# bmhopkinson/hyslam

Measured on AMD Instinct MI355X. Metric: stereo frames/sec ORB extract+match, 1920x1080 @2000 feat, higher is better.
Workload: dtype u8

## Files before the change

hyslam_amd/csrc/hs_api.hip:

```cpp
#include "hs_plan.h"
#include "hs_track.h"
#include <atomic>
#include <climits>
#include <cmath>
#include <cstdio>
#include <cstring>
#include <mutex>
#include <string>
#include <vector>

#define HS_VERSION "hyslam_amd 0.1 (gfx950)"

template <class T, bool Pinned = false> struct HsBuf {
    T* p = nullptr; size_t cap = 0;
    HsBuf() = default;
    HsBuf(const HsBuf&) = delete; HsBuf& operator=(const HsBuf&) = delete;
    HsBuf(HsBuf&& o) noexcept : p(o.p), cap(o.cap) { o.p = nullptr; o.cap = 0; }
    HsBuf& operator=(HsBuf&& o) noexcept { if (this != &o) { release(); p = o.p; cap = o.cap; o.p = nullptr; o.cap = 0; } return *this; }
    ~HsBuf() { release(); }
    void release() { if (p) (void)(Pinned ? hipHostFree(p) : hipFree(p)); p = nullptr; cap = 0; }
    hipError_t grow(size_t count)
    {
        if (count <= cap) return hipSuccess;
        release();
        const hipError_t e = Pinned ? hipHostMalloc((void**)&p, count * sizeof(T), hipHostMallocDefault) : hipMalloc((void**)&p, count * sizeof(T));
        if (e != hipSuccess) { p = nullptr; return e; }
        cap = count;
        return Pinned ? hipSuccess : hs_poison_fresh(p, count * sizeof(T));
    }
    hipError_t grow(size_t count, hipStream_t drain)
    {
        if (count <= cap) return hipSuccess;
        const hipError_t e = hipStreamSynchronize(drain);
        return e != hipSuccess ? e : grow(count);
    }
    operator T*() const { return p; }
};
template <class T> using HsPinned = HsBuf<T, true>;

struct HsFrameStaging { HsBuf<uint8_t> d_in, d_raw; };
struct HsStereoOut {
    HsBuf<float> ur, depth; HsBuf<int32_t> bd;
    hipError_t grow(size_t entries, hipStream_t drain)
    {
        if (entries <= ur.cap && entries <= depth.cap && entries <= bd.cap) return hipSuccess;
        hipError_t e = hipStreamSynchronize(drain);
        if (e == hipSuccess) e = ur.grow(entries);
        if (e == hipSuccess) e = depth.grow(entries);
        if (e == hipSuccess) e = bd.grow(entries);
        return e;
    }
};

struct hs_orb {
    hs_orb_params p;
    int device = 0;
    std::atomic<bool> owned{true};
    std::atomic<int> refs{1};
    hipStream_t stream = nullptr;
    std::string err;
    uint16_t taps[7];
    HsKnobs knobs{};
    uint32_t fast_epoch = 0;
    hipStream_t s_aux = nullptr; hipEvent_t ev_sfork = nullptr, ev_sjoin = nullptr;
    bool fast_taps = false;
    std::vector<float> scale, inv_scale, sigma2, inv_sigma2;
    std::vector<int> quota;
    struct Geometry {
        int w = 0, h = 0, batch_cap = 0;
        uint64_t plan_digest = 0;
        std::vector<HsLevel> lv;
        std::vector<HsLevel> lv_n;
        int last_batch = 0; HsImg0 last_img0{};
        int last_pyr_launches = 0;
        int total_cells = 0, max_wcell = 1, max_hcell = 1;
        int fast_items = 0;
        int fast_items_n = 0;
        uint64_t cand_img_stride = 0;
        int sel_img_stride = 0;
        int max_kp = 0;
        HsBuf<HsFastItem> d_fast_items, d_fast_items_n;
        HsBuf<uint32_t> d_fast_ovf;
        HsBuf<uint8_t> d_pyr;
// ... 123 lines not shown
    g.cand_img_stride = P.cand_img_stride; g.sel_img_stride = P.sel_img_stride; g.max_kp = P.max_kp;
    g.qhist_stride = P.qhist_stride; g.qbest_stride = P.qbest_stride; g.plan_digest = P.digest;
    g.lv = std::move(P.lv); g.lv_n = std::move(P.lv_n);
    g.pyr_fuse = std::move(P.pyr_fuse); g.pyr_chain = std::move(P.pyr_chain); g.pyr_deep = std::move(P.pyr_deep);
    g.pyr_fuse_cols = std::move(P.pyr_fuse_cols); g.pyr_chain_cols = std::move(P.pyr_chain_cols); g.pyr_deep_cols = std::move(P.pyr_deep_cols);
    g.pyr_level_cols = std::move(P.pyr_level_cols);

    HIP_TRY(h, g.d_pyr.grow(std::max<size_t>(P.pyr_per_img * batch, 256)));
    HIP_TRY(h, g.d_tables.grow(std::max<size_t>(P.tables.size(), 256 / sizeof(int16_t))));
    const size_t ce = std::max<uint64_t>(g.cand_img_stride * batch, 64);
    HIP_TRY(h, g.d_cand.grow(ce));
    HIP_TRY(h, g.d_pts_xy.grow(ce));
    HIP_TRY(h, g.d_pts_sk.grow(ce));
    HIP_TRY(h, g.d_pt_node.grow(ce));
    if (h->qt_large) HIP_TRY(h, g.d_qt_rects.grow((size_t)batch * L * hs_quadtree_large_scratch_bytes()));
    HIP_TRY(h, g.d_cell_count.grow(std::max<size_t>((size_t)g.total_cells * batch, 64 / 4)));
    HIP_TRY(h, g.d_cand_count.grow((size_t)batch * L));
    HIP_TRY(h, g.d_sel_count.grow((size_t)batch * L));
    HIP_TRY(h, g.d_sel.grow(std::max<size_t>((size_t)g.sel_img_stride * batch * 3, 64 / 4)));
    HIP_TRY(h, g.d_sel_perm.grow(std::max<size_t>((size_t)g.sel_img_stride * batch, 64 / 2)));
    HIP_TRY(h, g.d_qt_tabs.grow(std::max<size_t>(P.qt_tabs.size() + 16, 256)));
    HIP_TRY(h, g.d_qkeys.grow(std::max<size_t>(P.qkeys.size() + 16 / 2, 256 / 2)));
    HIP_TRY(h, g.d_fast_qt.grow(HS_MAX_LEVELS));
    HIP_TRY(h, g.d_qhist.grow(std::max<size_t>((size_t)g.qhist_stride * batch, 256 / 4)));
    HIP_TRY(h, g.d_qbest.grow(std::max<size_t>((size_t)g.qbest_stride * batch, 256 / 8)));
    HIP_TRY(h, g.d_pyr_tabs.grow(std::max<size_t>(P.pyr_tabs.size() * 8, 256)));
    HIP_TRY(h, g.d_pyr_cols.grow(std::max<size_t>(P.pyr_cols.size() * 8, 256)));
    HIP_TRY(h, g.d_fast_items.grow(P.items.size()));
    HIP_TRY(h, g.d_fast_items_n.grow(P.items_n.size()));
    HIP_TRY(h, g.d_fast_ovf.grow(std::max<size_t>(hs_fast_overflow_bytes(h->knobs, g.max_hcell, g.fast_items, g.fast_items_n, batch), 256) / 4));

    relocate_levels(g.lv, g); relocate_levels(g.lv_n, g);
    relocate_pyramid(g);
    for (size_t l = 0; l < P.fast_qt.size(); l++) if (P.fast_qt[l].enabled) { relocate(P.fast_qt[l].xkey, g.d_qkeys.p); relocate(P.fast_qt[l].ykey, g.d_qkeys.p); }
    for (std::vector<HsFastItem>* items : { &P.items, &P.items_n })
        for (HsFastItem& it : *items) if (it.level > 0) relocate(it.base, g.d_pyr.p);

    HIP_TRY(h, upload(g.d_tables, P.tables));
    HIP_TRY(h, upload(g.d_qt_tabs, P.qt_tabs));
    HIP_TRY(h, upload(g.d_qkeys, P.qkeys));
    HIP_TRY(h, upload(g.d_fast_qt, P.fast_qt));
    HIP_TRY(h, upload(g.d_pyr_tabs, P.pyr_tabs));
    HIP_TRY(h, upload(g.d_pyr_cols, P.pyr_cols));
    HIP_TRY(h, hipMemcpy(h->d_lv, g.lv.data(), sizeof(HsLevel) * L, hipMemcpyHostToDevice));
    HIP_TRY(h, hipMemcpy(h->d_lv + L, g.lv_n.data(), sizeof(HsLevel) * L, hipMemcpyHostToDevice));
    HIP_TRY(h, upload(g.d_fast_items, P.items));
    HIP_TRY(h, upload(g.d_fast_items_n, P.items_n));

    HIP_TRY(h, hipMemsetAsync(g.d_qhist, 0, std::max<size_t>((size_t)g.qhist_stride * batch * 4, 256), h->stream));
    HIP_TRY(h, hipMemsetAsync(g.d_qbest, 0, std::max<size_t>((size_t)g.qbest_stride * batch * 8, 256), h->stream));
    HIP_TRY(h, hipMemsetAsync(g.d_fast_ovf, 0, 4 * HS_FAST_QUEUE_DWORDS * 4, h->stream));
    HIP_TRY(h, hipStreamSynchronize(h->stream));
    g.w = w; g.h = hh; g.batch_cap = batch;
    return HS_OK;
}

enum KnobRule { K_ANY, K_FLAG , K_POSITIVE , K_NONNEG , K_MIN2 ,
                K_TRISTATE  };
struct KnobRow { const char* name; int HsKnobs::* field; int def; KnobRule rule; const char* meaning; };
const KnobRow KNOBS[] = {
    { "HS_PYRAMID_NO_FUSE",     &HsKnobs::no_fuse,             0,             K_FLAG,     "one pyramid level per launch (parity tests of the unfused kernel)" },
    { "HS_PYRAMID_CHAIN",       &HsKnobs::chain_mode,          -1,            K_ANY,      "-1 = a three-level chain for the tail of an odd number of levels, 0 = never, 2 = chains for every fused pair too (parity tests)" },
    { "HS_PYRAMID_CHAIN2",      &HsKnobs::pyr_chain2,          0,             K_FLAG,     "HS_PYRAMID_PLAN: a 2 is a two-level chain launch, not the two-level kernel" },
    { "HS_PYRAMID_TBX_MAX",     &HsKnobs::pyr_tbx_max,         0,             K_ANY,      "cap on the level-B tile width of the two-level kernel (experiment: lane utilisation against time)" },
    { "HS_PYRAMID_DEEP_MAX",    &HsKnobs::deep_max_batch,      2,             K_ANY,      "calls of at most this many frames use the small-batch plan (0 = never)" },
    { "HS_PYRAMID_DEEP_ROWS",   &HsKnobs::deep_rows,           8,             K_MIN2,     "rows of the LAST level per tile in the small-batch plan" },
    { "HS_FAST_ORDER",          &HsKnobs::fast_order,          1,             K_ANY,      "order of an image's FAST work items: 1 = reduced levels deepest first, level 0 last; 0 = level 0 first (the order until round 3); 2 = reduced levels interleaved, level 0 last" },
    { "HS_FAST_PCAP",           &HsKnobs::fast_pcap,           0,             K_ANY,      "tuning: cap on the FAST kernel's list length" },
    { "HS_FAST_LIST_MIN",       &HsKnobs::fast_list_min,       0,             K_ANY,      "tuning: list entries the tallest item must keep (decides the workgroups per CU; 1024 = round 4's layout)" },
    { "HS_FAST_TEST_SMALL_LISTS", &HsKnobs::fast_small_lists,  0,             K_FLAG,     "parity tests: force the spill paths" },
    { "HS_FAST_WG_PER_CU",      &HsKnobs::fast_wg_per_cu,      0,             K_ANY,      "tuning: workgroups per CU" },
    { "HS_FAST_TEST_SCAN_B",    &HsKnobs::fast_scan_b,         0,             K_FLAG,     "parity tests: NMS from the score tile" },
    { "HS_FAST_IMAGE_MAJOR",    &HsKnobs::fast_image_major,    0,             K_FLAG,     "tuning / parity tests: the work units image-major whatever the batch" },
    { "HS_FAST_NQ",             &HsKnobs::fast_nq,             0,             K_ANY,      "tuning / parity tests: at most this many work queues (8, 16, 32)" },
    { "HS_FAST_COLS",           &HsKnobs::fast_cols,           0,             K_ANY,      "tuning / parity tests: 32 / 64 = narrow / wide items whatever the batch (default: by batch)" },
    { "HS_FAST_NARROW_MAX",     &HsKnobs::fast_narrow_max,     0,             K_ANY,      "tuning: narrow items for launches of at most this many (narrow) work items" },
    { "HS_FAST_NO_FOLD",        &HsKnobs::fast_no_fold,        0,             K_FLAG,     "tuning / parity tests: work queues even for launches of <= 2 units per workgroup" },
    { "HS_FAST_KEYS",           &HsKnobs::fast_keys,           1,             K_FLAG,     "0: the quadtree kernel gathers the candidates and computes the keys itself (the scheme until round 3)" },
    { "HS_FAST_KEYS_LEVELS",    &HsKnobs::fast_keys_levels,    HS_MAX_LEVELS, K_POSITIVE, "only the levels 0 .. n-1 get keys (tuning)" },
    { "HS_FAST_KEYS_MAX_BATCH", &HsKnobs::fast_keys_max_batch, 16,            K_NONNEG,   "calls of more frames than this run without the keys (see run_extract)" },
    { "HS_QT_POINT_DOMAIN",     &HsKnobs::qt_point_domain,     0,             K_FLAG,     "the quadtree's general point-domain passes only (parity tests of the fallback)" },
    { "HS_QT_SMALL",            &HsKnobs::qt_small,            0,             K_FLAG,     "the quadtree kernel's small instance (two workgroups per CU) where every level's list fits it" },
    { "HS_STEREO_FUSE",         &HsKnobs::stereo_fuse,         1,             K_FLAG,     "0: the stereo front end with a separate k_stereo_strips launch instead of the strips binned by an extra workgroup of the describe launch" },
    { "HS_EXTRACT_SPLIT",       &HsKnobs::split_mode,          -1,            K_TRISTATE, "1 = always run level 0's FAST + quadtree beside the pyramid, 0 = never, unset = for small batches (hs_orb_set_split overrides)" },
};
}
HsKnobs hs_read_knobs()
{
    HsKnobs k{};
    for (const KnobRow& r : KNOBS) {
        int& dst = k.*r.field;
        dst = r.def;
        const char* e = getenv(r.name);
        if (!e) continue;
        const int v = atoi(e);
        switch (r.rule) {
        case K_ANY: dst = v; break;
        case K_FLAG: dst = v != 0; break;
        case K_POSITIVE: if (v > 0) dst = v; break;
        case K_NONNEG: if (v >= 0) dst = v; break;
        case K_MIN2: if (v >= 2) dst = v; break;
        case K_TRISTATE: dst = v == INT_MIN ? -1 : (v != 0 ? 1 : 0); break;
        }
    }
    if (const char* e = getenv("HS_PYRAMID_PLAN")) { k.pyr_plan_set = true; k.pyr_plan = e; }
    return k;
}
namespace {

struct OutLayout { size_t off_k, off_d, off_u, off_z, bytes; };
OutLayout out_layout(int batch, int cap, int pairs)
{
    OutLayout o;
    o.off_k = hs_up256((size_t)batch * 4);
    o.off_d = o.off_k + hs_up256((size_t)batch * cap * sizeof(hs_keypoint));
    const size_t desc = (size_t)batch * cap * HS_DESC_BYTES, ur = (size_t)pairs * cap * 4;
    o.off_u = o.off_z = o.bytes = o.off_d + desc;
    if (pairs > 0) { o.off_u = o.off_d + hs_up256(desc); o.off_z = o.off_u + hs_up256(ur); o.bytes = o.off_z + ur; }
    return o;
}

void scatter_results(const uint8_t* blk, const OutLayout& o, int batch, int cap0, int pairs, hs_keypoint* kps, uint8_t* desc, int32_t* n, int cap, float* uRight, float* depth)
{
    memcpy(n, blk, (size_t)batch * 4);
    for (int i = 0; i < batch; i++) {
        const size_t cnt = (size_t)std::min(std::max(n[i], 0), cap0);
        memcpy(kps + (size_t)i * cap, blk + o.off_k + (size_t)i * cap0 * sizeof(hs_keypoint), cnt * sizeof(hs_keypoint));
        memcpy(desc + (size_t)i * cap * HS_DESC_BYTES, blk + o.off_d + (size_t)i * cap0 * HS_DESC_BYTES, cnt * HS_DESC_BYTES);
        if (i < pairs) {
            memcpy(uRight + (size_t)i * cap, blk + o.off_u + (size_t)i * cap0 * 4, cnt * 4);
            memcpy(depth + (size_t)i * cap, blk + o.off_z + (size_t)i * cap0 * 4, cnt * 4);
        }
    }
}

int ensure_stereo_strips(hs_orb* h, int pairs, int cap, int n_rows)
{
    if (n_rows > 65536) return hs_fail(h, HS_ERR_INVALID, "stereo: more than 65536 image rows");
    const size_t need_count = (size_t)pairs * hs_stereo_strips(n_rows);
    HIP_TRY(h, h->d_strip_count.grow(need_count, h->stream));
    HIP_TRY(h, h->d_strip_list.grow(need_count * (size_t)cap, h->stream));
    return HS_OK;
}

int run_extract(hs_orb* h, HsImg0 img0, int batch, HsOut out, hipStream_t s, const HsStripFuse* sf = nullptr)
{
    const int L = h->p.nlevels;
    hs_orb::Geometry& g = h->geo;
    const bool narrow = hs_fast_narrow(h->knobs, g.fast_items_n, batch);
    const HsPyrChain* const deep = (batch <= h->knobs.deep_max_batch && !g.pyr_deep.empty()) ? g.pyr_deep.data() : nullptr;
    const bool use_keys = h->knobs.fast_keys && g.d_fast_qt.p != nullptr && batch <= h->knobs.fast_keys_max_batch;
    if (g.keys_dirty) {
        HIP_TRY(h, hipDeviceSynchronize());
        if (g.d_qhist) HIP_TRY(h, hipMemsetAsync(g.d_qhist, 0, (size_t)g.qhist_stride * g.batch_cap * 4, s));
        if (g.d_qbest) HIP_TRY(h, hipMemsetAsync(g.d_qbest, 0, (size_t)g.qbest_stride * g.batch_cap * 8, s));
        HIP_TRY(h, hipStreamSynchronize(s));
        g.keys_dirty = false;
    }
    if (use_keys) g.keys_dirty = true;
    const std::vector<HsLevel>& lvh = narrow ? h->geo.lv_n : h->geo.lv;
    const HsLevel* const d_lv = h->d_lv + (narrow ? L : 0);
    const HsFastItem* const d_items = narrow ? g.d_fast_items_n.p : g.d_fast_items.p;
    const int n_items = narrow ? g.fast_items_n : g.fast_items;
    const int items0 = lvh[0].ngroups * lvh[0].nrows, first0 = lvh[0].item_begin;
    const bool split = !h->prof && L > 1 && items0 > 0 && items0 < n_items && (h->knobs.split_mode == 1 || (h->knobs.split_mode < 0 && batch <= 2 && (size_t)g.w * (size_t)g.h * (size_t)batch >= 6000000));
    auto fast = [&](int item_first, int item_count, int spill_slot, hipStream_t st) -> int {
        const HsFastLaunch plan = hs_fast_launch_plan(h->knobs, g.max_hcell, g.fast_items, g.fast_items_n, batch, item_first, item_count, spill_slot);
        const bool launched = hs_launch_fast(plan, d_items, img0, h->p.fast_threshold, g.d_cand, g.d_cell_count, g.cand_img_stride, g.total_cells, g.d_fast_ovf, h->fast_epoch,
                                             use_keys ? g.d_fast_qt.p : nullptr, g.d_qhist, g.d_qbest, g.qhist_stride, g.qbest_stride, st);
        const hipError_t e = hipGetLastError();
        if (e != hipSuccess) {
            (void)hipDeviceSynchronize();
            (void)hipMemsetAsync(g.d_fast_ovf, 0, 4 * HS_FAST_QUEUE_DWORDS * 4, h->stream);
            if (g.d_qhist) (void)hipMemsetAsync(g.d_qhist, 0, (size_t)g.qhist_stride * g.batch_cap * 4, h->stream);
            if (g.d_qbest) (void)hipMemsetAsync(g.d_qbest, 0, (size_t)g.qbest_stride * g.batch_cap * 8, h->stream);
            (void)hipStreamSynchronize(h->stream);
            return hs_fail(h, HS_ERR_HIP, std::string("FAST launch: ") + hipGetErrorString(e));
        }
        if (launched) h->fast_epoch++;
        return HS_OK;
    };
    auto quadtree = [&](int level_first, int level_count, hipStream_t st) {
        hs_launch_quadtree(d_lv, L, batch, g.total_cells, g.d_cand, g.d_cell_count, g.cand_img_stride,
                           g.d_pts_xy, g.d_pts_sk, g.d_pt_node, g.d_cand_count, g.d_sel, g.d_sel_count, g.sel_img_stride, g.d_sel_perm, h->knobs.qt_point_domain ? 1 : 0,
                           level_first, level_count, use_keys ? g.d_qhist.p : nullptr, g.d_qbest, g.qhist_stride, g.qbest_stride, h->keep_points ? 1 : 0,
                           h->qt_large ? 2 : (h->qt_small_ok ? 1 : 0), g.d_qt_rects, st);
    };
    if (split) {
        if (!h->s_aux) {
            HIP_TRY(h, hipStreamCreateWithFlags(&h->s_aux, hipStreamNonBlocking));
            HIP_TRY(h, hipEventCreateWithFlags(&h->ev_sfork, hipEventDisableTiming));
            HIP_TRY(h, hipEventCreateWithFlags(&h->ev_sjoin, hipEventDisableTiming));
        }
        HIP_TRY(h, hipEventRecord(h->ev_sfork, s));
        HIP_TRY(h, hipStreamWaitEvent(h->s_aux, h->ev_sfork, 0));
        int rc = fast(first0, items0, 1, h->s_aux);
        if (rc != HS_OK) return rc;
        quadtree(0, 1, h->s_aux);
        HIP_TRY(h, hipEventRecord(h->ev_sjoin, h->s_aux));
        h->geo.last_pyr_launches = hs_launch_pyramid(h->d_lv, h->geo.lv.data(), g.pyr_fuse.data(), g.pyr_chain.data(), L, img0, batch, s, HsPyrCols{ g.pyr_fuse_cols.data(), g.pyr_chain_cols.data(), g.pyr_deep_cols.data(), g.pyr_level_cols.data() }, deep);
        rc = fast(0, n_items - items0, 0, s);
        if (rc != HS_OK) return rc;
        quadtree(1, L - 1, s);
        HIP_TRY(h, hipStreamWaitEvent(s, h->ev_sjoin, 0));
    } else {
        mark(h, 0, s);
        h->geo.last_pyr_launches = hs_launch_pyramid(h->d_lv, h->geo.lv.data(), g.pyr_fuse.data(), g.pyr_chain.data(), L, img0, batch, s, HsPyrCols{ g.pyr_fuse_cols.data(), g.pyr_chain_cols.data(), g.pyr_deep_cols.data(), g.pyr_level_cols.data() }, deep);
        mark(h, 1, s);
        const int rc = fast(0, n_items, 0, s);
        if (rc != HS_OK) return rc;
        mark(h, 2, s);
        quadtree(0, L, s);
    }
    mark(h, 3, s);
    hs_launch_describe(h->d_lv, L, img0, batch, g.d_sel, g.d_sel_count, g.d_sel_perm, g.sel_img_stride, g.max_kp,
                       h->d_taps, out, s, h->fast_taps, sf ? *sf : HsStripFuse{});
    mark(h, -1, s);
    HIP_TRY(h, hipGetLastError());
    g.keys_dirty = false;
    h->geo.last_batch = batch; h->geo.last_img0 = img0;
    return HS_OK;
}

struct DevFrame { hs_keypoint* kps; uint8_t* desc; int8_t* cell; };
void stage_frame(HsStage& st, const hs_frame_view* F, DevFrame* o)
{
    st.in(&o->kps, F->n, F->kps); st.in(&o->desc, (size_t)F->n * 32, F->desc);
    st.temp(&o->cell, hs_frame_grid_bytes(std::max(F->n, 1)));
}

void run_stereo(hs_orb* h, bool binned, const hs_keypoint* kL, const uint8_t* dL, const int32_t* nL, const hs_keypoint* kR, const uint8_t* dR,
                const int32_t* nR, int pairs, int cap, const hs_stereo_params& sp, float* ur, float* depth, hipStream_t s)
{
    mark(h, 4, s);
    h->last_stereo_launches = binned ? 1 : 2;
    if (binned) hs_launch_stereo_match_only(kL, dL, nL, kR, dR, nR, pairs, cap, sp, ur, depth, h->st.bd, h->d_strip_count, h->d_strip_list, s);
    else hs_launch_stereo(kL, dL, nL, kR, dR, nR, pairs, cap, sp, ur, depth, h->st.bd, h->d_strip_count, h->d_strip_list, s);
    mark(h, 5, s);
    hs_launch_stereo_median(nL, pairs, cap, ur, depth, h->st.bd, sp.th_high, h->d_strip_count, sp.n_rows, s);
    mark(h, -1, s);
}

int run_stereo_frontend(hs_orb* h, HsImg0 img0, HsOut out, const hs_stereo_params& sp, float* ur, float* depth, hipStream_t s)
{
    const int pairs = out.split;
    const HsStripFuse sf{ 1, sp.n_rows, hs_stereo_strips(sp.n_rows), 0, sp.size_ref, h->d_strip_count, h->d_strip_list };
    const int rc = run_extract(h, img0, 2 * pairs, out, s, h->knobs.stereo_fuse ? &sf : nullptr);
    if (rc != HS_OK) return rc;
    run_stereo(h, h->knobs.stereo_fuse, out.kps, out.desc, out.n, out.kps2, out.desc2, out.n2, pairs, out.cap, sp, ur, depth, s);
    HIP_TRY(h, hipGetLastError());
    return HS_OK;
}

template <class Body> int run_lanes(hs_orb* h, hipStream_t s, int count, Body body)
{
    hs_orb* const child = h->lane2;
    const int c0 = count / 2;
    child->prof = h->prof;
    HIP_TRY(h, hipEventRecord(h->ev_fork, s));
    HIP_TRY(h, hipStreamWaitEvent(child->stream, h->ev_fork, 0));
    int rc = body(h, 0, c0, s);
    if (rc == HS_OK) {
        rc = body(child, c0, count - c0, child->stream);
        if (rc != HS_OK) h->err = child->err;
    }
    HIP_TRY(h, hipEventRecord(h->ev_join, child->stream));
    HIP_TRY(h, hipStreamWaitEvent(s, h->ev_join, 0));
    return rc;
}

}

void hs_debug_plan_summary(const hs_orb* h, int32_t* out )
{
    for (int i = 0; i < 8; i++) out[i] = 0;
    if (!h || h->geo.lv.empty()) return;
    const int L = h->p.nlevels;
    out[0] = hs_pyramid_launch_count(h->geo.lv.data(), L);
    int deep_launches = 0, longest = 0, lds = 0;
    for (int l = 1; l < L; l++) {
        deep_launches++;
        if (l < (int)h->geo.pyr_deep.size() && h->geo.pyr_deep[l].valid) {
            const HsPyrChain& C = h->geo.pyr_deep[l];
            if (C.nstage > longest) { longest = C.nstage; lds = (int)hs_pyr_chain_lds((size_t)C.x_bytes, C.h_rows); }
            l += C.nstage - 1;
        } else if (h->geo.lv[l].chain_n > 0 && l + h->geo.lv[l].chain_n <= L) l += h->geo.lv[l].chain_n - 1;
        else if (h->geo.lv[l].fuse_tbx > 0 && l + 1 < L) l++;
    }
    out[1] = L > 1 ? deep_launches : 0; out[2] = h->geo.fast_items; out[3] = h->geo.fast_items_n;
    for (int l = 0; l < L; l++) out[4] += h->geo.lv[l].qt_hist_off != 0xFFFFFFFFu;
    out[5] = longest; out[6] = lds;
    if (L > 1 && !h->geo.pyr_deep.empty() && h->geo.pyr_deep[1].valid) out[7] = h->geo.pyr_deep[1].grid_x * h->geo.pyr_deep[1].grid_y;
}
void hs_debug_pyramid_plan(const hs_orb* h, HsDebugPyramidPlan* out)
{
    *out = HsDebugPyramidPlan{};
    if (!h || h->geo.w <= 0) return;
    out->nlevels = h->p.nlevels; out->lv = h->geo.lv.data();
    out->fuse = h->geo.pyr_fuse.data(); out->chain = h->geo.pyr_chain.data(); out->deep = h->geo.pyr_deep.data();
    out->cols = HsPyrCols{ h->geo.pyr_fuse_cols.data(), h->geo.pyr_chain_cols.data(), h->geo.pyr_deep_cols.data(), h->geo.pyr_level_cols.data() };
}
uint64_t hs_debug_plan_digest(const hs_orb* h) { return h && h->geo.w > 0 ? h->geo.plan_digest : 0; }

std::atomic<int> g_hs_poison{-1};
static std::atomic<long long> g_hs_poison_violations{0};
void hs_poison_violation() { g_hs_poison_violations.fetch_add(1, std::memory_order_relaxed); }
hipError_t hs_poison_fill(void* p, size_t bytes, int byte)
{
    const hipError_t e = hipMemset(p, byte, bytes);
    return e != hipSuccess ? e : hipStreamSynchronize(nullptr);
}
__global__ __launch_bounds__(256) void k_poison_check(const uint8_t* __restrict__ base, const HsPoisonGaps g, int byte, unsigned long long* __restrict__ first)
{
    const int gap = blockIdx.x;
    if (gap >= g.n) return;
    const unsigned long long e = g.end[gap];
    unsigned long long m = ~0ull;
    for (unsigned long long i = g.begin[gap] + threadIdx.x; i < e; i += 256)
        if (base[i] != (uint8_t)byte) { m = i; break; }
    if (m != ~0ull) atomicMin(first + gap, m);
// ... 1272 lines not shown
```

hyslam_amd/csrc/hs_plan.h:

```cpp
#pragma once
#include "hs_internal.h"

struct HsKnobs {
    int no_fuse, stereo_fuse, fast_keys, fast_keys_levels, fast_keys_max_batch, fast_order;
    int fast_pcap, fast_list_min, fast_small_lists, fast_wg_per_cu, fast_scan_b, fast_image_major, fast_nq, fast_cols, fast_narrow_max, fast_no_fold;
    int chain_mode, pyr_chain2, pyr_tbx_max, deep_max_batch, deep_rows;
    int qt_point_domain, qt_small, split_mode;
    bool pyr_plan_set = false;
    std::string pyr_plan;
};
HsKnobs hs_read_knobs();

struct HsPlanInput {
    const hs_orb_params* p;
    const float* inv_scale; const float* scale; const int* quota;
    const HsKnobs* knobs;
    bool qt_large;
    int w, h;
};

struct HsPlan {
    int w = 0, h = 0;
    int total_cells = 0, max_wcell = 1, max_hcell = 1, fast_items = 0, fast_items_n = 0;
    uint64_t cand_img_stride = 0; int sel_img_stride = 0, max_kp = 0;
    uint32_t qhist_stride = 0, qbest_stride = 0;
    size_t pyr_per_img = 0;
    std::vector<HsLevel> lv, lv_n;
    std::vector<int16_t> tables;
    std::vector<uint8_t> qt_tabs;
    std::vector<uint16_t> qkeys;
    std::vector<HsFastQt> fast_qt;
    std::vector<uint64_t> pyr_tabs;
    std::vector<uint64_t> pyr_cols;
    std::vector<HsPyrFuseCols> pyr_fuse_cols;
    std::vector<HsPyrChainCols> pyr_chain_cols, pyr_deep_cols;
    std::vector<HsPyrFuse> pyr_fuse;
    std::vector<HsPyrChain> pyr_chain;
    std::vector<HsPyrChain> pyr_deep;
    std::vector<const uint8_t*> pyr_level_cols;
    std::vector<HsFastItem> items, items_n;
    uint64_t digest = 0;
};

int hs_plan_geometry(const HsPlanInput& in, HsPlan& out, std::string& err);
void hs_plan_pyramid(const HsKnobs& k, HsPlan& P);
const char* hs_plan_fast_items(const HsKnobs& k, HsPlan& P);
uint64_t hs_plan_digest(const HsPlan& P);
```

hyslam_amd/csrc/kernels_stereo.hip:

```cpp
#define SM_DIST_TH_HIGH 257
#include "hs_internal.h"

#define STRIP_SHIFT HS_STRIP_SHIFT

#define STRIPS_T 1024
#define STRIPS_MAX HS_STRIPS_MAX
__global__ __launch_bounds__(STRIPS_T) void k_stereo_strips(const hs_keypoint* __restrict__ kpsR, const int32_t* __restrict__ nRs, int cap,
                                                            float size_ref, int n_rows, int n_strips,
                                                            int32_t* __restrict__ strip_count, HsStripEntry* __restrict__ strip_list)
{
    __shared__ int s_cnt[STRIPS_MAX];
    const int pair = blockIdx.x, tid = threadIdx.x;
    const int nR = min(nRs[pair], cap);
    for (int s = tid; s < n_strips; s += STRIPS_T) s_cnt[s] = 0;
    constexpr int KPT = 4;
    __syncthreads();
    for (int i0 = 0; i0 < nR; i0 += STRIPS_T * KPT) {
        float kx[KPT], ky[KPT], ks[KPT]; int ko[KPT];
#pragma unroll
        for (int k = 0; k < KPT; k++) {
            const int i = min(i0 + tid + STRIPS_T * k, nR - 1);
            const hs_keypoint* kr = &kpsR[(size_t)pair * cap + i];
            kx[k] = kr->x; ky[k] = kr->y; ks[k] = kr->size; ko[k] = kr->octave;
        }
#pragma unroll
        for (int k = 0; k < KPT; k++) {
            const int i = i0 + tid + STRIPS_T * k;
            if (i >= nR) continue;
            const float r = 2.0f * ks[k] / size_ref;
            int maxr = (int)ceilf(ky[k] + r), minr = (int)floorf(ky[k] - r);
            if (maxr < 0 || minr >= n_rows) continue;
            minr = max(minr, 0); maxr = min(maxr, n_rows - 1);
            for (int s = minr >> STRIP_SHIFT; s <= (maxr >> STRIP_SHIFT); s++) {
                const int slot = atomicAdd(&s_cnt[s], 1);
                const int lo = max(minr - (s << STRIP_SHIFT), 0), hi = min(maxr - (s << STRIP_SHIFT), 31);
                HsStripEntry e; e.uR = kx[k]; e.octave = ko[k]; e.idx_band = (uint32_t)i | ((uint32_t)lo << 16) | ((uint32_t)hi << 24); e._pad = 0;
                strip_list[((size_t)pair * n_strips + s) * cap + slot] = e;
            }
        }
    }
    __syncthreads();
    for (int s = tid; s < n_strips; s += STRIPS_T) strip_count[(size_t)pair * n_strips + s] = s_cnt[s];
}

template <int SM_KPW>
__global__ __launch_bounds__(256) void k_stereo_match(const int32_t* __restrict__ strip_count, const HsStripEntry* __restrict__ strip_list, int n_strips,
                                                      const hs_keypoint* __restrict__ kpsL, const uint8_t* __restrict__ descL,
                                                      const int32_t* __restrict__ nLs,
                                                      const hs_keypoint* __restrict__ kpsR, const uint8_t* __restrict__ descR,
                                                      const int32_t* __restrict__ nRs,
                                                      int cap, hs_stereo_params sp,
                                                      float* __restrict__ uRight, float* __restrict__ depth, int32_t* __restrict__ best_dist)
{
    const int lane = threadIdx.x & 63, wv = __builtin_amdgcn_readfirstlane(threadIdx.x >> 6);
    const int pair = blockIdx.y;
    const int iL0 = (blockIdx.x * 4 + wv) * SM_KPW;
    const int nL = min(nLs[pair], cap);
    if (iL0 >= cap) return;
    const size_t o = (size_t)pair * cap;
    const float mbf = sp.mbf, mb = sp.mbf / sp.fx;
    const float minD = 0.f, maxD = mbf / mb;
    const float th_high = sp.th_high;

    float uL[SM_KPW], minU[SM_KPW], maxU[SM_KPW]; int levelL[SM_KPW], rowIn[SM_KPW], nc[SM_KPW];
    const HsStripEntry* cl[SM_KPW]; const unsigned long long* dl[SM_KPW];
    bool live[SM_KPW];
    int ncmax = 0;
#pragma unroll
    for (int t = 0; t < SM_KPW; t++) {
        const int iL = iL0 + t;
        live[t] = iL < nL;
        const hs_keypoint kl = kpsL[o + min(iL, max(nL - 1, 0))];
        const float vL = kl.y;
        uL[t] = kl.x; levelL[t] = kl.octave;
        minU[t] = uL[t] - maxD; maxU[t] = uL[t] - minD;
        const int rowL = (int)vL;
        const bool ok = live[t] && (vL >= 0.f) && rowL < sp.n_rows && !(maxU[t] < 0.f);
        const size_t sb = (size_t)pair * n_strips + (ok ? (rowL >> STRIP_SHIFT) : 0);
        nc[t] = ok ? strip_count[sb] : 0;
        cl[t] = strip_list + sb * cap;
        rowIn[t] = rowL & 31;
        dl[t] = reinterpret_cast<const unsigned long long*>(descL + (o + min(iL, max(nL - 1, 0))) * 32);
        ncmax = max(ncmax, nc[t]);
    }
    uint32_t best[SM_KPW];
#pragma unroll
    for (int t = 0; t < SM_KPW; t++) best[t] = 0xFFFFFFFFu;
    for (int c0 = 0; c0 < ncmax; c0 += 128) {
        HsStripEntry e[SM_KPW][2]; bool pass[SM_KPW][2];
#pragma unroll
        for (int t = 0; t < SM_KPW; t++)
#pragma unroll
            for (int j = 0; j < 2; j++) {
                const int c = c0 + 64 * j + lane;
                pass[t][j] = c < nc[t];
                e[t][j] = cl[t][pass[t][j] ? c : 0];
            }
#pragma unroll
        for (int t = 0; t < SM_KPW; t++)
#pragma unroll
            for (int j = 0; j < 2; j++) {
                const int lo = (int)((e[t][j].idx_band >> 16) & 0xFFu), hi = (int)(e[t][j].idx_band >> 24);
                pass[t][j] = pass[t][j] && !(rowIn[t] < lo || rowIn[t] > hi);
                pass[t][j] = pass[t][j] && !(e[t][j].octave < levelL[t] - 1 || e[t][j].octave > levelL[t] + 1);
                pass[t][j] = pass[t][j] && (e[t][j].uR >= minU[t] && e[t][j].uR <= maxU[t]);
            }
        unsigned long long dr[SM_KPW][2][4];
#pragma unroll
        for (int t = 0; t < SM_KPW; t++)
#pragma unroll
            for (int j = 0; j < 2; j++) {
                const unsigned long long* p = reinterpret_cast<const unsigned long long*>(descR + (o + (e[t][j].idx_band & 0xFFFFu)) * 32);
                if (pass[t][j]) { dr[t][j][0] = p[0]; dr[t][j][1] = p[1]; dr[t][j][2] = p[2]; dr[t][j][3] = p[3]; }
                else { dr[t][j][0] = dr[t][j][1] = dr[t][j][2] = dr[t][j][3] = 0ull; }
            }
#pragma unroll
        for (int t = 0; t < SM_KPW; t++) {
            const unsigned long long l0 = dl[t][0], l1 = dl[t][1], l2 = dl[t][2], l3 = dl[t][3];
#pragma unroll
            for (int j = 0; j < 2; j++) {
                const int d = __popcll(l0 ^ dr[t][j][0]) + __popcll(l1 ^ dr[t][j][1]) + __popcll(l2 ^ dr[t][j][2]) + __popcll(l3 ^ dr[t][j][3]);
                if (pass[t][j] && (float)d < th_high) best[t] = min(best[t], ((uint32_t)d << 16) | (e[t][j].idx_band & 0xFFFFu));
            }
        }
    }
#pragma unroll
    for (int t = 0; t < SM_KPW; t++) {
#pragma unroll
        for (int s = 32; s > 0; s >>= 1) best[t] = min(best[t], (uint32_t)__shfl_xor((int)best[t], s, 64));
        bool rowHasCandidates = false;
        if (best[t] == 0xFFFFFFFFu && sp.th_high < (sp.th_high + sp.th_low) / 2) {
            bool hit = false;
            for (int c = lane; c < nc[t]; c += 64) {
                const uint32_t ib = cl[t][c].idx_band;
                hit = hit || !(rowIn[t] < (int)((ib >> 16) & 0xFFu) || rowIn[t] > (int)(ib >> 24));
            }
            rowHasCandidates = __ballot(hit) != 0ull;
        }
        const int iL = iL0 + t;
        if (iL >= cap) break;
        if (lane == 0) {
            float ur_out = -1.0f, depth_out = -1.0f; int bd = -1;
            if (live[t] && (best[t] != 0xFFFFFFFFu || rowHasCandidates)) {
                const bool found = best[t] != 0xFFFFFFFFu;
                const float bestDist = found ? (float)(best[t] >> 16) : th_high;
                const int bestIdxR = found ? (int)(best[t] & 0xFFFF) : 0;
                const float dist_threshold = (sp.th_high + sp.th_low) / 2;
                if (bestDist < dist_threshold) {
                    float uR0 = kpsR[o + bestIdxR].x;
                    float disparity = uL[t] - uR0;
                    if (disparity >= minD && disparity < maxD) {
                        if (disparity <= 0) { disparity = 0.01; uR0 = uL[t] - 0.01; }
                        depth_out = mbf / disparity;
                        ur_out = uR0;
                        bd = found ? (int)(best[t] >> 16) : SM_DIST_TH_HIGH;
                    }
                }
            }
            uRight[o + iL] = ur_out; depth[o + iL] = depth_out; best_dist[o + iL] = bd;
        }
    }
}

__global__ __launch_bounds__(256) void k_stereo_median(const int32_t* __restrict__ nLs, int cap,
                                                       float* __restrict__ uRight, float* __restrict__ depth,
                                                       const int32_t* __restrict__ best_dist, float th_high,
                                                       int32_t* __restrict__ strip_count, int n_strips)
{
    __shared__ int hist[258];
    __shared__ float s_th;
    const int pair = blockIdx.x;
    const int nL = min(nLs[pair], cap);
    const size_t o = (size_t)pair * cap;
    for (int i = threadIdx.x; i < 258; i += 256) hist[i] = 0;
    __syncthreads();
    constexpr int DPT = 8;
    int dreg[DPT];
#pragma unroll
    for (int k = 0; k < DPT; k++) { const int i = threadIdx.x + 256 * k; dreg[k] = i < nL ? best_dist[o + i] : -1; }
#pragma unroll
    for (int k = 0; k < DPT; k++) if (dreg[k] >= 0) atomicAdd(&hist[min(dreg[k], 257)], 1);
    for (int i = threadIdx.x + 256 * DPT; i < nL; i += 256) {
        int d = best_dist[o + i];
        if (d >= 0) atomicAdd(&hist[min(d, 257)], 1);
    }
    __syncthreads();
    if (threadIdx.x < 64) {
        const int lane = threadIdx.x;
        const int b0 = hist[4 * lane], b1 = hist[4 * lane + 1], b2 = hist[4 * lane + 2], b3 = hist[4 * lane + 3];
        int incl = b0 + b1 + b2 + b3;
#pragma unroll
        for (int s = 1; s < 64; s <<= 1) { const int v = __shfl_up(incl, s, 64); if (lane >= s) incl += v; }
        const int below256 = __shfl(incl, 63, 64), total = below256 + hist[256] + hist[257];
        const int target = total / 2, excl = incl - (b0 + b1 + b2 + b3);
        int med = -1;
        if (excl <= target && incl > target) med = 4 * lane + (excl + b0 > target ? 0 : excl + b0 + b1 > target ? 1 : excl + b0 + b1 + b2 > target ? 2 : 3);
        const unsigned long long hit = __ballot(med >= 0);
        if (total == 0) { if (lane == 0) s_th = -1.f; }
        else if (hit == 0) { if (lane == 0) s_th = 1.5f * 1.4f * (below256 + hist[256] > target ? 256.f : th_high); }
        else if (med >= 0) s_th = 1.5f * 1.4f * (float)med;
    }
    __syncthreads();
    const float th = s_th;
    if (th < 0.f) return;
#pragma unroll
    for (int k = 0; k < DPT; k++) {
        const int i = threadIdx.x + 256 * k, d = dreg[k];
        if (d >= 0 && (d == SM_DIST_TH_HIGH ? !(th_high < th) : !((float)d < th))) { uRight[o + i] = -1.f; depth[o + i] = -1.f; }
    }
    for (int i = threadIdx.x + 256 * DPT; i < nL; i += 256) {
        int d = best_dist[o + i];
        if (d >= 0 && (d == SM_DIST_TH_HIGH ? !(th_high < th) : !((float)d < th))) { uRight[o + i] = -1.f; depth[o + i] = -1.f; }
    }
}

void hs_launch_stereo(const hs_keypoint* kpsL, const uint8_t* descL, const int32_t* nL,
                      const hs_keypoint* kpsR, const uint8_t* descR, const int32_t* nR,
                      int pairs, int cap, hs_stereo_params sp, float* uRight, float* depth, int32_t* best_dist,
                      int32_t* strip_count, void* strip_list, hipStream_t s)
{
    if (pairs <= 0 || cap <= 0) return;
    HsStripEntry* const sl = reinterpret_cast<HsStripEntry*>(strip_list);
    const int n_strips = hs_stereo_strips(sp.n_rows);
    hipLaunchKernelGGL(k_stereo_strips, dim3(pairs), dim3(STRIPS_T), 0, s, kpsR, nR, cap, sp.size_ref, sp.n_rows, n_strips, strip_count, sl);
    if ((size_t)pairs * cap >= (size_t)8 * 2048) {
        dim3 grid((cap + 7) / 8, pairs, 1);
        hipLaunchKernelGGL(k_stereo_match<2>, grid, dim3(256), 0, s, strip_count, sl, n_strips, kpsL, descL, nL, kpsR, descR, nR, cap, sp, uRight, depth, best_dist);
    } else {
        dim3 grid((cap + 3) / 4, pairs, 1);
        hipLaunchKernelGGL(k_stereo_match<1>, grid, dim3(256), 0, s, strip_count, sl, n_strips, kpsL, descL, nL, kpsR, descR, nR, cap, sp, uRight, depth, best_dist);
    }
}

void hs_launch_stereo_median(const int32_t* nL, int pairs, int cap, float* uRight, float* depth, const int32_t* best_dist, float th_high,
                             int32_t* strip_count, int n_rows, hipStream_t s)
{
    if (pairs <= 0 || cap <= 0) return;
    hipLaunchKernelGGL(k_stereo_median, dim3(pairs), dim3(256), 0, s, nL, cap, uRight, depth, best_dist, th_high, strip_count, hs_stereo_strips(n_rows));
}

void hs_launch_stereo_match_only(const hs_keypoint* kpsL, const uint8_t* descL, const int32_t* nL,
                                 const hs_keypoint* kpsR, const uint8_t* descR, const int32_t* nR,
                                 int pairs, int cap, hs_stereo_params sp, float* uRight, float* depth, int32_t* best_dist,
                                 const int32_t* strip_count, const void* strip_list, hipStream_t s)
{
    if (pairs <= 0 || cap <= 0) return;
    const HsStripEntry* const sl = reinterpret_cast<const HsStripEntry*>(strip_list);
    const int n_strips = hs_stereo_strips(sp.n_rows);
    if ((size_t)pairs * cap >= (size_t)8 * 2048) {
        dim3 grid((cap + 7) / 8, pairs, 1);
        hipLaunchKernelGGL(k_stereo_match<2>, grid, dim3(256), 0, s, strip_count, sl, n_strips, kpsL, descL, nL, kpsR, descR, nR, cap, sp, uRight, depth, best_dist);
    } else {
        dim3 grid((cap + 3) / 4, pairs, 1);
        hipLaunchKernelGGL(k_stereo_match<1>, grid, dim3(256), 0, s, strip_count, sl, n_strips, kpsL, descL, nL, kpsR, descR, nR, cap, sp, uRight, depth, best_dist);
    }
}
```

Before: 48940.

## Add wave-compacted stereo matcher handling several left keypoints per wavefront

```diff
diff --git a/hyslam_amd/csrc/hs_api.hip b/hyslam_amd/csrc/hs_api.hip
--- a/hyslam_amd/csrc/hs_api.hip
+++ b/hyslam_amd/csrc/hs_api.hip
@@ -1,4 +1,5 @@
 #include "hs_plan.h"
+#include "hs_stereo.h"
 #include "hs_track.h"
 #include <atomic>
 #include <climits>
@@ -288,7 +289,8 @@
     { "HS_QT_POINT_DOMAIN",     &HsKnobs::qt_point_domain,     0,             K_FLAG,     "the quadtree's general point-domain passes only (parity tests of the fallback)" },
     { "HS_QT_SMALL",            &HsKnobs::qt_small,            0,             K_FLAG,     "the quadtree kernel's small instance (two workgroups per CU) where every level's list fits it" },
     { "HS_STEREO_FUSE",         &HsKnobs::stereo_fuse,         1,             K_FLAG,     "0: the stereo front end with a separate k_stereo_strips launch instead of the strips binned by an extra workgroup of the describe launch" },
-    { "HS_EXTRACT_SPLIT",       &HsKnobs::split_mode,          -1,            K_TRISTATE, "1 = always run level 0's FAST + quadtree beside the pyramid, 0 = never, unset = for small batches (hs_orb_set_split overrides)" },
+    { "HS_STEREO_KPW",          &HsKnobs::stereo_kpw,          0,             K_ANY,      "tuning / parity tests: left keypoints per wavefront of the stereo matcher: 0 = by batch, 1 / 2 = k_stereo_match, 4 / 8 = k_stereo_match_compact, whatever the batch" },
+    { "HS_EXTRACT_SPLIT",       &HsKnobs::split_mode,         -1,            K_TRISTATE, "1 = always run level 0's FAST + quadtree beside the pyramid, 0 = never, unset = for small batches (hs_orb_set_split overrides)" },
 };
 }
 HsKnobs hs_read_knobs()
@@ -440,8 +442,8 @@
 {
     mark(h, 4, s);
     h->last_stereo_launches = binned ? 1 : 2;
-    if (binned) hs_launch_stereo_match_only(kL, dL, nL, kR, dR, nR, pairs, cap, sp, ur, depth, h->st.bd, h->d_strip_count, h->d_strip_list, s);
-    else hs_launch_stereo(kL, dL, nL, kR, dR, nR, pairs, cap, sp, ur, depth, h->st.bd, h->d_strip_count, h->d_strip_list, s);
+    if (binned) hs_launch_stereo_match_only_kpw(kL, dL, nL, kR, dR, nR, pairs, cap, sp, ur, depth, h->st.bd, h->d_strip_count, h->d_strip_list, h->knobs.stereo_kpw, s);
+    else hs_launch_stereo_kpw(kL, dL, nL, kR, dR, nR, pairs, cap, sp, ur, depth, h->st.bd, h->d_strip_count, h->d_strip_list, h->knobs.stereo_kpw, s);
     mark(h, 5, s);
     hs_launch_stereo_median(nL, pairs, cap, ur, depth, h->st.bd, sp.th_high, h->d_strip_count, sp.n_rows, s);
     mark(h, -1, s);
diff --git a/hyslam_amd/csrc/hs_plan.h b/hyslam_amd/csrc/hs_plan.h
--- a/hyslam_amd/csrc/hs_plan.h
+++ b/hyslam_amd/csrc/hs_plan.h
@@ -2,7 +2,7 @@
 #include "hs_internal.h"
 
 struct HsKnobs {
-    int no_fuse, stereo_fuse, fast_keys, fast_keys_levels, fast_keys_max_batch, fast_order;
+    int no_fuse, stereo_fuse, stereo_kpw, fast_keys, fast_keys_levels, fast_keys_max_batch, fast_order;
     int fast_pcap, fast_list_min, fast_small_lists, fast_wg_per_cu, fast_scan_b, fast_image_major, fast_nq, fast_cols, fast_narrow_max, fast_no_fold;
     int chain_mode, pyr_chain2, pyr_tbx_max, deep_max_batch, deep_rows;
     int qt_point_domain, qt_small, split_mode;
diff --git a/hyslam_amd/csrc/hs_stereo.h b/hyslam_amd/csrc/hs_stereo.h
--- /dev/null
+++ b/hyslam_amd/csrc/hs_stereo.h
@@ -0,0 +1,12 @@
+#pragma once
+
+int hs_stereo_kpw(int knob, int pairs, int cap);
+
+void hs_launch_stereo_kpw(const hs_keypoint* kpsL, const uint8_t* descL, const int32_t* nL,
+                          const hs_keypoint* kpsR, const uint8_t* descR, const int32_t* nR,
+                          int pairs, int cap, hs_stereo_params sp, float* uRight, float* depth, int32_t* best_dist,
+                          int32_t* strip_count, void* strip_list, int kpw_knob, hipStream_t s);
+void hs_launch_stereo_match_only_kpw(const hs_keypoint* kpsL, const uint8_t* descL, const int32_t* nL,
+                                     const hs_keypoint* kpsR, const uint8_t* descR, const int32_t* nR,
+                                     int pairs, int cap, hs_stereo_params sp, float* uRight, float* depth, int32_t* best_dist,
+                                     const int32_t* strip_count, const void* strip_list, int kpw_knob, hipStream_t s);
diff --git a/hyslam_amd/csrc/kernels_stereo.hip b/hyslam_amd/csrc/kernels_stereo.hip
--- a/hyslam_amd/csrc/kernels_stereo.hip
+++ b/hyslam_amd/csrc/kernels_stereo.hip
@@ -1,5 +1,6 @@
 #define SM_DIST_TH_HIGH 257
 #include "hs_internal.h"
+#include "hs_stereo.h"
 
 #define STRIP_SHIFT HS_STRIP_SHIFT
 
@@ -162,6 +163,132 @@
     }
 }
 
+#define SMC_QCAP 192
+#define SMC_FENCE() __builtin_amdgcn_fence(__ATOMIC_SEQ_CST, "wavefront")
+__device__ __forceinline__ int smc_wave_append(bool flag, int& base)
+{
+    const unsigned long long m = __ballot(flag);
+    const int slot = base + (int)__builtin_amdgcn_mbcnt_hi((unsigned)(m >> 32), __builtin_amdgcn_mbcnt_lo((unsigned)m, 0u));
+    base += (int)__popcll(m);
+    return slot;
+}
+template <int K>
+__global__ __launch_bounds__(256) void k_stereo_match_compact(const int32_t* __restrict__ strip_count, const HsStripEntry* __restrict__ strip_list, int n_strips,
+                                                              const hs_keypoint* __restrict__ kpsL, const uint8_t* __restrict__ descL,
+                                                              const int32_t* __restrict__ nLs,
+                                                              const hs_keypoint* __restrict__ kpsR, const uint8_t* __restrict__ descR,
+                                                              const int32_t* __restrict__ nRs,
+                                                              int cap, hs_stereo_params sp,
+                                                              float* __restrict__ uRight, float* __restrict__ depth, int32_t* __restrict__ best_dist)
+{
+    static_assert(K >= 2 && K <= 16 && (K & (K - 1)) == 0, "K keypoint records and 4 K descriptor words fit the lanes of a wave");
+    __shared__ uint32_t s_queue[4][SMC_QCAP];
+    __shared__ __attribute__((aligned(16))) unsigned long long s_descL[4][K][4];
+    __shared__ uint32_t s_best[4][K];
+    const int lane = threadIdx.x & 63, wv = __builtin_amdgcn_readfirstlane(threadIdx.x >> 6);
+    const int pair = blockIdx.y;
+    const int iL0 = (blockIdx.x * 4 + wv) * K;
+    if (iL0 >= cap) return;
+    const int nL = min(nLs[pair], cap);
+    const size_t o = (size_t)pair * cap;
+    const float mbf = sp.mbf, mb = sp.mbf / sp.fx;
+    const float minD = 0.f, maxD = mbf / mb;
+    const float th_high = sp.th_high;
+    uint32_t* const queue = s_queue[wv];
+
+    const int iL = iL0 + min(lane, K - 1);
+    const bool live = iL < nL;
+    const hs_keypoint kl = kpsL[o + min(iL, max(nL - 1, 0))];
+    const float vL = kl.y, uL = kl.x;
+    const int levelL = kl.octave;
+    const float minU = uL - maxD, maxU = uL - minD;
+    const int rowL = (int)vL;
+    const bool ok = live && (vL >= 0.f) && rowL < sp.n_rows && !(maxU < 0.f);
+    const int sb = pair * n_strips + (ok ? (rowL >> STRIP_SHIFT) : 0);
+    const int nc = ok ? strip_count[sb] : 0;
+    const int rowIn = rowL & 31;
+    if (lane < 4 * K) {
+        const int il = iL0 + (lane >> 2);
+        s_descL[wv][lane >> 2][lane & 3] = reinterpret_cast<const unsigned long long*>(descL + (o + min(il, max(nL - 1, 0))) * 32)[lane & 3];
+    }
+    if (lane < K) s_best[wv][lane] = 0xFFFFFFFFu;
+    SMC_FENCE();
+
+    auto hamming = [&](int qi, bool act) {
+        const uint32_t q = act ? queue[qi] : 0u;
+        const int tq = (int)(q >> 16), iR = (int)(q & 0xFFFFu);
+        if (act) {
+            const unsigned long long* p = reinterpret_cast<const unsigned long long*>(descR + (o + iR) * 32);
+            const unsigned long long r0 = p[0], r1 = p[1], r2 = p[2], r3 = p[3];
+            const ulonglong2 la = *reinterpret_cast<const ulonglong2*>(&s_descL[wv][tq][0]), lb = *reinterpret_cast<const ulonglong2*>(&s_descL[wv][tq][2]);
+            const int d = __popcll(la.x ^ r0) + __popcll(la.y ^ r1) + __popcll(lb.x ^ r2) + __popcll(lb.y ^ r3);
+            if ((float)d < th_high) atomicMin(&s_best[wv][tq], ((uint32_t)d << 16) | (uint32_t)iR);
+        }
+    };
+
+    int qn = 0;
+    uint32_t band_mask = 0;
+#pragma nounroll
+    for (int t = 0; t < K; t++) {
+        const int nc_t = __builtin_amdgcn_readlane(nc, t);
+        if (nc_t == 0) continue;
+        const HsStripEntry* const cl = strip_list + (size_t)__builtin_amdgcn_readlane(sb, t) * cap;
+        const int rowIn_t = __builtin_amdgcn_readlane(rowIn, t), levelL_t = __builtin_amdgcn_readlane(levelL, t);
+        const float minU_t = __int_as_float(__builtin_amdgcn_readlane(__float_as_int(minU), t));
+        const float maxU_t = __int_as_float(__builtin_amdgcn_readlane(__float_as_int(maxU), t));
+        for (int c0 = 0; c0 < nc_t; c0 += 128) {
+            HsStripEntry e[2]; bool band[2], pass[2];
+#pragma unroll
+            for (int j = 0; j < 2; j++) {
+                const int c = c0 + 64 * j + lane;
+                band[j] = c < nc_t;
+                e[j] = cl[band[j] ? c : 0];
+            }
+#pragma unroll
+            for (int j = 0; j < 2; j++) {
+                const int lo = (int)((e[j].idx_band >> 16) & 0xFFu), hi = (int)(e[j].idx_band >> 24);
+                band[j] = band[j] && !(rowIn_t < lo || rowIn_t > hi);
+                pass[j] = band[j] && !(e[j].octave < levelL_t - 1 || e[j].octave > levelL_t + 1);
+                pass[j] = pass[j] && (e[j].uR >= minU_t && e[j].uR <= maxU_t);
+            }
+            if (__ballot(band[0] || band[1]) != 0ull) band_mask |= 1u << t;
+#pragma unroll
+            for (int j = 0; j < 2; j++) {
+                const int slot = smc_wave_append(pass[j], qn);
+                if (pass[j]) queue[slot] = ((uint32_t)t << 16) | (e[j].idx_band & 0xFFFFu);
+            }
+            SMC_FENCE();
+            while (qn >= 64) { qn -= 64; hamming(qn + lane, true); }
+            SMC_FENCE();
+        }
+    }
+    if (qn > 0) hamming(lane, lane < qn);
+    SMC_FENCE();
+
+    if (lane < K && iL < cap) {
+        const uint32_t best = s_best[wv][lane];
+        const bool rowHasCandidates = best == 0xFFFFFFFFu && sp.th_high < (sp.th_high + sp.th_low) / 2 && ((band_mask >> lane) & 1u) != 0;
+        float ur_out = -1.0f, depth_out = -1.0f; int bd = -1;
+        if (live && (best != 0xFFFFFFFFu || rowHasCandidates)) {
+            const bool found = best != 0xFFFFFFFFu;
+            const float bestDist = found ? (float)(best >> 16) : th_high;
+            const int bestIdxR = found ? (int)(best & 0xFFFF) : 0;
+            const float dist_threshold = (sp.th_high + sp.th_low) / 2;
+            if (bestDist < dist_threshold) {
+                float uR0 = kpsR[o + bestIdxR].x;
+                float disparity = uL - uR0;
+                if (disparity >= minD && disparity < maxD) {
+                    if (disparity <= 0) { disparity = 0.01; uR0 = uL - 0.01; }
+                    depth_out = mbf / disparity;
+                    ur_out = uR0;
+                    bd = found ? (int)(best >> 16) : SM_DIST_TH_HIGH;
+                }
+            }
+        }
+        uRight[o + iL] = ur_out; depth[o + iL] = depth_out; best_dist[o + iL] = bd;
+    }
+}
+
 __global__ __launch_bounds__(256) void k_stereo_median(const int32_t* __restrict__ nLs, int cap,
                                                        float* __restrict__ uRight, float* __restrict__ depth,
                                                        const int32_t* __restrict__ best_dist, float th_high,
@@ -214,22 +341,47 @@
     }
 }
 
+#define HS_STEREO_COMPACT4_MIN_SLOTS ((size_t)6 * 2048)
+#define HS_STEREO_COMPACT8_MIN_SLOTS ((size_t)24 * 2048)
+int hs_stereo_kpw(int knob, int pairs, int cap)
+{
+    if (knob == 1 || knob == 2 || knob == 4 || knob == 8) return knob;
+    const size_t slots = (size_t)pairs * cap;
+    return slots >= HS_STEREO_COMPACT8_MIN_SLOTS ? 8 : slots >= HS_STEREO_COMPACT4_MIN_SLOTS ? 4 : 1;
+}
+
+namespace {
+void launch_match(int kpw, const int32_t* strip_count, const HsStripEntry* sl, int n_strips, const hs_keypoint* kpsL, const uint8_t* descL, const int32_t* nL,
+                  const hs_keypoint* kpsR, const uint8_t* descR, const int32_t* nR, int pairs, int cap, hs_stereo_params sp, float* uRight, float* depth,
+                  int32_t* best_dist, hipStream_t s)
+{
+    const dim3 grid((cap + 4 * kpw - 1) / (4 * kpw), pairs, 1);
+#define SM_LAUNCH(KERNEL) hipLaunchKernelGGL(KERNEL, grid, dim3(256), 0, s, strip_count, sl, n_strips, kpsL, descL, nL, kpsR, descR, nR, cap, sp, uRight, depth, best_dist)
+    if (kpw == 8) SM_LAUNCH(k_stereo_match_compact<8>);
+    else if (kpw == 4) SM_LAUNCH(k_stereo_match_compact<4>);
+    else if (kpw == 2) SM_LAUNCH(k_stereo_match<2>);
+    else SM_LAUNCH(k_stereo_match<1>);
+#undef SM_LAUNCH
+}
+}
+
+void hs_launch_stereo_kpw(const hs_keypoint* kpsL, const uint8_t* descL, const int32_t* nL,
+                          const hs_keypoint* kpsR, const uint8_t* descR, const int32_t* nR,
+                          int pairs, int cap, hs_stereo_params sp, float* uRight, float* depth, int32_t* best_dist,
+                          int32_t* strip_count, void* strip_list, int kpw_knob, hipStream_t s)
+{
+    if (pairs <= 0 || cap <= 0) return;
+    HsStripEntry* const sl = reinterpret_cast<HsStripEntry*>(strip_list);
+    const int n_strips = hs_stereo_strips(sp.n_rows);
+    hipLaunchKernelGGL(k_stereo_strips, dim3(pairs), dim3(STRIPS_T), 0, s, kpsR, nR, cap, sp.size_ref, sp.n_rows, n_strips, strip_count, sl);
+    launch_match(hs_stereo_kpw(kpw_knob, pairs, cap), strip_count, sl, n_strips, kpsL, descL, nL, kpsR, descR, nR, pairs, cap, sp, uRight, depth, best_dist, s);
+}
 void hs_launch_stereo(const hs_keypoint* kpsL, const uint8_t* descL, const int32_t* nL,
                       const hs_keypoint* kpsR, const uint8_t* descR, const int32_t* nR,
                       int pairs, int cap, hs_stereo_params sp, float* uRight, float* depth, int32_t* best_dist,
                       int32_t* strip_count, void* strip_list, hipStream_t s)
 {
-    if (pairs <= 0 || cap <= 0) return;
-    HsStripEntry* const sl = reinterpret_cast<HsStripEntry*>(strip_list);
-    const int n_strips = hs_stereo_strips(sp.n_rows);
-    hipLaunchKernelGGL(k_stereo_strips, dim3(pairs), dim3(STRIPS_T), 0, s, kpsR, nR, cap, sp.size_ref, sp.n_rows, n_strips, strip_count, sl);
-    if ((size_t)pairs * cap >= (size_t)8 * 2048) {
-        dim3 grid((cap + 7) / 8, pairs, 1);
-        hipLaunchKernelGGL(k_stereo_match<2>, grid, dim3(256), 0, s, strip_count, sl, n_strips, kpsL, descL, nL, kpsR, descR, nR, cap, sp, uRight, depth, best_dist);
-    } else {
-        dim3 grid((cap + 3) / 4, pairs, 1);
-        hipLaunchKernelGGL(k_stereo_match<1>, grid, dim3(256), 0, s, strip_count, sl, n_strips, kpsL, descL, nL, kpsR, descR, nR, cap, sp, uRight, depth, best_dist);
-    }
+    hs_launch_stereo_kpw(kpsL, descL, nL, kpsR, descR, nR, pairs, cap, sp, uRight, depth, best_dist, strip_count, strip_list, 0, s);
 }
 
 void hs_launch_stereo_median(const int32_t* nL, int pairs, int cap, float* uRight, float* depth, const int32_t* best_dist, float th_high,
@@ -239,19 +391,19 @@
     hipLaunchKernelGGL(k_stereo_median, dim3(pairs), dim3(256), 0, s, nL, cap, uRight, depth, best_dist, th_high, strip_count, hs_stereo_strips(n_rows));
 }
 
+void hs_launch_stereo_match_only_kpw(const hs_keypoint* kpsL, const uint8_t* descL, const int32_t* nL,
+                                     const hs_keypoint* kpsR, const uint8_t* descR, const int32_t* nR,
+                                     int pairs, int cap, hs_stereo_params sp, float* uRight, float* depth, int32_t* best_dist,
+                                     const int32_t* strip_count, const void* strip_list, int kpw_knob, hipStream_t s)
+{
+    if (pairs <= 0 || cap <= 0) return;
+    launch_match(hs_stereo_kpw(kpw_knob, pairs, cap), strip_count, reinterpret_cast<const HsStripEntry*>(strip_list), hs_stereo_strips(sp.n_rows), kpsL, descL, nL,
+                 kpsR, descR, nR, pairs, cap, sp, uRight, depth, best_dist, s);
+}
 void hs_launch_stereo_match_only(const hs_keypoint* kpsL, const uint8_t* descL, const int32_t* nL,
                                  const hs_keypoint* kpsR, const uint8_t* descR, const int32_t* nR,
                                  int pairs, int cap, hs_stereo_params sp, float* uRight, float* depth, int32_t* best_dist,
                                  const int32_t* strip_count, const void* strip_list, hipStream_t s)
 {
-    if (pairs <= 0 || cap <= 0) return;
-    const HsStripEntry* const sl = reinterpret_cast<const HsStripEntry*>(strip_list);
-    const int n_strips = hs_stereo_strips(sp.n_rows);
-    if ((size_t)pairs * cap >= (size_t)8 * 2048) {
-        dim3 grid((cap + 7) / 8, pairs, 1);
-        hipLaunchKernelGGL(k_stereo_match<2>, grid, dim3(256), 0, s, strip_count, sl, n_strips, kpsL, descL, nL, kpsR, descR, nR, cap, sp, uRight, depth, best_dist);
-    } else {
-        dim3 grid((cap + 3) / 4, pairs, 1);
-        hipLaunchKernelGGL(k_stereo_match<1>, grid, dim3(256), 0, s, strip_count, sl, n_strips, kpsL, descL, nL, kpsR, descR, nR, cap, sp, uRight, depth, best_dist);
-    }
-}
+    hs_launch_stereo_match_only_kpw(kpsL, descL, nL, kpsR, descR, nR, pairs, cap, sp, uRight, depth, best_dist, strip_count, strip_list, 0, s);
+}
```

New measurement: 49500 (median of 6 runs). 1.01x the previous value.
